# rahul-rwat/ESMStereo

Measured on AMD Instinct MI355X. Metric: stereo pairs/sec at 384×1248 maxdisp=192; EPE vs reference, higher is better.
Workload: dtype f32; 1 GPU; hot path: cost volume -> 3D stems -> 3D hourglass -> regression -> ESM upsampler (models/ESMStereo.py:700-745), ESMStereo-S gwc 384x1248 md192 B1; variant=S, cv=gwc, global_batch=1, height=384, width=1248, maxdisp=192, parallelism=dp1, graph=True

## Files before the change

### esmstereo_amd/blocks.py

```python
from __future__ import annotations

from typing import List, Optional, Sequence, Tuple

import torch
import torch.nn as nn
import torch.nn.functional as F

from .engine import (ACT_GELU, ACT_NONE, CONVT1X1_PAIRED, FORK_ENABLED, SC11_ENABLED, Ctx, PackedConv,
                     convt_1x1_supported, eager_emit, forked_packs, pack_conv, pack_shuffle_tail, pair2_auto,
                     param_token, run_conv, run_conv_forked, run_convt_1x1, run_pair2, run_shuffle_conv,
                     run_shuffle_tail, run_side_partial, shuffle_conv_pre_supported, shuffle_conv_supported)
from .mixer import FMBlock

__all__ = ["BasicConv", "Conv2x", "aggregation", "up_refinement", "upsample4", "upsample8", "upsample16"]


class BasicConv(nn.Module):

    def __init__(self, in_channels: int, out_channels: int, deconv: bool = False, is_3d: bool = False,
                 bn: bool = True, gelu: bool = True, **kwargs) -> None:
        super().__init__()
        self.gelu = gelu
        self.use_bn = bn
        kinds = {(False, False): nn.Conv2d, (False, True): nn.ConvTranspose2d,
                 (True, False): nn.Conv3d, (True, True): nn.ConvTranspose3d}
        self.conv = kinds[(bool(is_3d), bool(deconv))](in_channels, out_channels, bias=False, **kwargs)
        self.bn = (nn.BatchNorm3d if is_3d else nn.BatchNorm2d)(out_channels)
        self._esm = None

    def packed(self) -> PackedConv:
        tok = param_token(self.conv, self.bn) + (self.use_bn, self.gelu)
        if self._esm is None or self._esm[0] != tok:
            self._esm = (tok, pack_conv(self.conv, self.bn if self.use_bn else None,
                                        ACT_GELU if self.gelu else ACT_NONE))
        return self._esm[1]

    def emit(self, ctx: Ctx, srcs: Sequence[torch.Tensor], **epi) -> torch.Tensor:
        return run_conv(ctx, self.packed(), srcs, tag=getattr(self, "_esm_name", "BasicConv"), **epi)

    def forward(self, x: torch.Tensor) -> torch.Tensor:
        return self.emit(Ctx(x.device), [x])


class Conv2x(nn.Module):

    def __init__(self, in_channels: int, out_channels: int, deconv: bool = False, is_3d: bool = False,
                 concat: bool = True, keep_concat: bool = True, bn: bool = True, gelu: bool = True,
                 keep_dispc: bool = False) -> None:
        super().__init__()
        self.concat = concat
        self.is_3d = is_3d
        if deconv and is_3d and keep_dispc:
            self.conv1 = BasicConv(in_channels, out_channels, deconv, is_3d, bn=True, gelu=True,
                                   kernel_size=(1, 4, 4), stride=(1, 2, 2), padding=(0, 1, 1))
        else:
            k = (4 if not is_3d else (4, 4, 4)) if deconv else 3
            self.conv1 = BasicConv(in_channels, out_channels, deconv, is_3d, bn=True, gelu=True, kernel_size=k,
                                   stride=2, padding=1)
        mul = (2 if keep_concat else 1) if concat else 1
        cin2 = out_channels * 2 if concat else out_channels
        self.conv2 = BasicConv(cin2, out_channels * mul, False, is_3d, bn, gelu, kernel_size=3, stride=1, padding=1)

    def forward(self, x: torch.Tensor, rem: torch.Tensor) -> torch.Tensor:
        x = self.conv1(x)
        if x.shape != rem.shape:
            x = F.interpolate(x, size=(rem.shape[-2], rem.shape[-1]), mode="nearest")
        if self.concat:
            return self.conv2.emit(Ctx(x.device), [x, rem]) if x.shape[1] % 4 == 0 and rem.shape[1] % 4 == 0 \
                else self.conv2(torch.cat((x, rem), 1))
        return self.conv2(x + rem)


def _bc(cin: int, cout: int, is_3d: bool, k: int = 3, s: int = 1, p: int = 1, **kw) -> BasicConv:
    return BasicConv(cin, cout, is_3d=is_3d, kernel_size=k, stride=s, padding=p, **kw)


def _up(cin: int, cout: int, is_3d: bool, last: bool = False) -> BasicConv:
    return BasicConv(cin, cout, deconv=True, is_3d=is_3d, bn=not last, gelu=not last, kernel_size=4, padding=1,
                     stride=2)


def _pair(ctx: Ctx, first: BasicConv, srcs: Sequence[torch.Tensor], second, second_packed: Optional[PackedConv] = None,
          regress: Optional[torch.Tensor] = None, **kw) -> torch.Tensor:
    n0 = getattr(first, "_esm_name", "BasicConv")
    n1 = getattr(second, "_esm_name", "conv") if second is not None else "conv"
    pb = second_packed if second_packed is not None else second.packed()
    if not kw:
        return run_pair2(ctx, first.packed(), srcs, pb, tags=(n0, n1), regress=regress)
    if regress is not None:
        raise ValueError("_pair: regress with an epilogue")
    mid = run_conv(ctx, first.packed(), srcs, tag=n0)
    return run_conv(ctx, pb, [mid], tag=n1, **kw)


def _crop_like(t: torch.Tensor, ref: torch.Tensor) -> torch.Tensor:
    idx = (slice(None), slice(None)) + tuple(slice(0, n) for n in ref.shape[2:])
    return t[idx]


class _Hourglass(nn.Module):

    is_3d = False

    def _build(self, c_in: int, c1: int, c2: int, c3: int, cat0: int, cat1: int) -> None:
        d3 = self.is_3d
        self.conv1 = nn.Sequential(_bc(c_in, c1, d3, s=2), _bc(c1, c1, d3))
        self.conv2 = nn.Sequential(_bc(c1, c2, d3, s=2), _bc(c2, c2, d3))
        self.conv3 = nn.Sequential(_bc(c2, c3, d3, s=2), _bc(c3, c3, d3))
        self.conv3_up = _up(c3, c2, d3)
        self.conv2_up = _up(c2, c1, d3)
        self.conv1_up = _up(c1, 1, d3, last=True)
        self.agg_0 = nn.Sequential(_bc(cat0, c2, d3, k=1, p=0), _bc(c2, c2, d3))
        self.agg_1 = nn.Sequential(_bc(cat1, c1, d3, k=1, p=0), _bc(c1, c1, d3))

    def _emit(self, ctx: Ctx, x: Optional[torch.Tensor], extra0: Sequence[torch.Tensor] = (),
              extra1: Sequence[torch.Tensor] = (), crop1: bool = True, c10: Optional[torch.Tensor] = None,
              c11: Optional[torch.Tensor] = None, **last) -> torch.Tensor:
        if c11 is not None:
            c1 = c11
        elif c10 is not None:
            c1 = self.conv1[1].emit(ctx, [c10])
        else:
            c1 = _pair(ctx, self.conv1[0], [x], self.conv1[1])
        c2 = _pair(ctx, self.conv2[0], [c1], self.conv2[1])
        c3 = _pair(ctx, self.conv3[0], [c2], self.conv3[1])
        a0 = self._up_agg(ctx, self.conv3_up, c3, self.agg_0, [c2, *extra0], True)
        a1 = self._up_agg(ctx, self.conv2_up, a0, self.agg_1, [c1, *extra1], crop1)
        return self.conv1_up.emit(ctx, [a1], **last)

    def _up_agg(self, ctx: Ctx, up: BasicConv, x: torch.Tensor, agg: nn.Sequential, skip: Sequence[torch.Tensor],
                crop: bool) -> torch.Tensor:
        ref = skip[0]
        if not crop and tuple(2 * v for v in x.shape[2:]) != tuple(ref.shape[2:]):
            raise RuntimeError(f"Sizes of tensors must match except in dimension 1. Expected size "
                               f"{2 * x.shape[2]} but got size {ref.shape[2]} for tensor number 1 in the list.")
        pa, pb = up.packed(), agg[0].packed()
        u_shape = tuple(2 * v for v in x.shape[2:])
        n0 = getattr(up, "_esm_name", "convT")
        n1 = getattr(agg[0], "_esm_name", "agg.0")
        paired = pair2_auto(pb, agg[1].packed(), [ref]) if not self.is_3d else False
        fork = FORK_ENABLED and not self.is_3d and len(skip) == 2 and agg[0].use_bn and int(skip[0].shape[1]) % 4 == 0
        if fork:
            cm = pa.cout + int(skip[0].shape[1])
            p_side, p_main = forked_packs(agg[0], agg[0].conv, agg[0].bn, ACT_GELU if agg[0].gelu else ACT_NONE, cm,
                                          int(skip[1].shape[1]))
            if convt_1x1_supported(pa, p_main, skip[:1]) and all(u >= r for u, r in zip(u_shape, ref.shape[2:])):
                part = run_side_partial(ctx, p_side, skip[1], n1, cm)
                h = run_convt_1x1(ctx, pa, [x], p_main, skip[:1], tags=(n0, n1), pre=part)
                ctx.meta[-1]["split"] = (0, cm)
                return agg[1].emit(ctx, [h])
            u = _crop_like(up.emit(ctx, [x]), ref)
            part = run_side_partial(ctx, p_side, skip[1], n1, cm)
            h = run_conv(ctx, p_main, [u, skip[0]], pre=part, tag=n1)
            ctx.meta[-1].update(layer=n1, split=(0, cm))
            return agg[1].emit(ctx, [h])
        if convt_1x1_supported(pa, pb, skip) and all(u >= r for u, r in zip(u_shape, ref.shape[2:])) and \
                (CONVT1X1_PAIRED or not paired):
            h = run_convt_1x1(ctx, pa, [x], pb, skip, tags=(n0, n1))
            return agg[1].emit(ctx, [h])
        u = _crop_like(up.emit(ctx, [x]), ref)
        return _pair(ctx, agg[0], [u, *skip], agg[1])


class aggregation(_Hourglass):

    is_3d = True

    def __init__(self, in_channels: int, add_channel: int) -> None:
        super().__init__()
        c0, a = in_channels, add_channel
        self._build(c0, c0 + a, c0 + 2 * a, c0 + 4 * a, 2 * (c0 + 2 * a), 2 * (c0 + a))

    def emit(self, ctx: Ctx, x: torch.Tensor, **last) -> torch.Tensor:
        return self._emit(ctx, x, crop1=True, **last)

    def forward(self, x: torch.Tensor) -> torch.Tensor:
        return eager_emit(x.device, self.emit, x)


class up_refinement(_Hourglass):

    is_3d = False

    def __init__(self, C: int, cf1: int, cf2: int) -> None:
        super().__init__()
        self._build(1, C, C, C, 2 * C + cf1, 2 * C + cf2)

    def emit(self, ctx: Ctx, disp: Optional[torch.Tensor], left_f1x: torch.Tensor, left_f2x: torch.Tensor,
             c10: Optional[torch.Tensor] = None, c11: Optional[torch.Tensor] = None, **last) -> torch.Tensor:
        return self._emit(ctx, disp, extra0=[left_f1x], extra1=[left_f2x], crop1=False, c10=c10, c11=c11, **last)

    def forward(self, disp: torch.Tensor, left_f1x: torch.Tensor, left_f2x: torch.Tensor) -> torch.Tensor:
        return eager_emit(disp.device, self.emit, disp, left_f1x, left_f2x)




def _dm(c: int) -> nn.Sequential:
    return nn.Sequential(_bc(1, c, False, k=5), _bc(c, c, False), _bc(c, c, False), _bc(c, c, False, k=1, p=1))


def _spx(cin: int, c: int, cout: int) -> nn.Sequential:
    return nn.Sequential(_bc(cin, c, False), nn.Conv2d(c, cout, 3, 1, 1, bias=False), nn.BatchNorm2d(cout), nn.GELU())


def _shuffle_up(nf: int, r: int) -> nn.Sequential:
    return nn.Sequential(nn.Conv2d(nf, nf * r * r, 1, 1, 0), nn.PixelShuffle(r), nn.SiLU(inplace=True))


class _ESMUpsampler(nn.Module):

    STAGES: Tuple = ()
    N_FEATS = 8

    def __init__(self) -> None:
        super().__init__()
        nf = self.N_FEATS
        for i, (tag, C, catc, spx_out, r, cf1, cf2, *_src) in enumerate(self.STAGES):
            setattr(self, f"dm{tag}", _dm(C))
            setattr(self, f"spx_{tag}", _spx(C + catc, C, spx_out))
            if i == 0:
                self.to_feat = nn.Conv2d(C, nf, 3, 1, 1, bias=False)
                self.blocks = nn.Sequential(*[FMBlock(nf, 7, 2) for _ in range(2)])
            setattr(self, f"upsampling{tag[:-1]}", _shuffle_up(nf, r))
            setattr(self, f"tail{tag}", nn.Conv2d(nf, 1, 3, 1, 1))
            setattr(self, f"ref{tag}", up_refinement(C, cf1, cf2))
        self._esm = None

    def _packed(self):
        tok = param_token(*self.modules())
        if self._esm is None or self._esm[0] != tok:
            p = {"to_feat": pack_conv(self.to_feat)}
            for (tag, _C, _cat, _spx, r, *_r) in self.STAGES:
                spx = getattr(self, f"spx_{tag}")
                p[f"spx1_{tag}"] = pack_conv(spx[1], spx[2], ACT_GELU)
                p[f"up_{tag}"] = pack_shuffle_tail(getattr(self, f"upsampling{tag[:-1]}")[0], getattr(self, f"tail{tag}"),
                                                   r)
            self._esm = (tok, p)
        return self._esm[1]

    def emit(self, ctx: Ctx, feats: Sequence[torch.Tensor], init_disp: torch.Tensor, final_scale: float = 1.0,
             scaled_copies: Optional[float] = None, init_cost: Optional[torch.Tensor] = None) -> List[torch.Tensor]:
        p = self._packed()
        me = getattr(self, "_esm_name", "upsample")
# ... 88 lines not shown
```

### esmstereo_amd/csrc/conv_pair2.hip

```cpp
#include "conv_direct.h"

namespace esm {
namespace conv {
namespace {

constexpr int kP2Threads = 256;
constexpr int kHintPairReg = 1 << 29;

__device__ __forceinline__ float regress_px(const float* __restrict__ cp, int D, int sc) {
#pragma clang fp contract(off)
    float acc = 0.f;
    for (int d0 = 0; d0 < D; d0 += 16) {
        float v[16];
#pragma unroll
        for (int k = 0; k < 16; ++k) v[k] = d0 + k < D ? cp[(d0 + k) * sc] : 0.f;
#pragma unroll
        for (int k = 0; k < 16; ++k)
            if (d0 + k < D) acc = acc + v[k] * static_cast<float>(d0 + k);
    }
    return acc;
}

template <int KA, int SA, int KB, int TH>
struct P2Geo {
// ... 185 lines not shown
        const bool ok = yb < bd.Ho && xb < bd.Wo && n < VB;
        const __amdgpu_buffer_rsrc_t ro = __builtin_amdgcn_make_buffer_rsrc(
            bd.out + b * bd.ob, static_cast<short>(0),
            4 * ((bd.Cout - 1) * static_cast<int>(bd.oc) + (bd.Ho - 1) * static_cast<int>(bd.oh) + bd.Wo), 0x00020000);
#pragma unroll
        for (int j = 0; j < 4; ++j) {
            const int co = 4 * kq + j;
            const float v = act_t<ESM_ACT_GELU>((acc[0][j] + acc[1][j]) * ep[32 + co] + ep[48 + co], 0);
            const unsigned o = (ok && co < bd.Cout) ? 4u * (co * static_cast<int>(bd.oc) + yb * static_cast<int>(bd.oh) + xb)
                                                    : kOOB;
            store_b32(__float_as_uint(v), ro, static_cast<int>(o), 0);
        }
    }
}

template <int KA, int SA, int KB, int TH, int CINMAX, bool REG = false>
int launch_p2(const esm_conv_desc& a, const esm_conv_desc& b, hipStream_t s) {
    using G = P2Geo<KA, SA, KB, TH>;
    const size_t lds = sizeof(float) * (static_cast<size_t>(CINMAX) * G::ICS + KA * KA * CINMAX * 16 + KB * KB * 256 +
                                        16 * G::ACS + 64);
    constexpr int VB = 16 - KB + 1;
    const dim3 grid(ceil_div(b.Wo, VB), ceil_div(b.Ho, TH), a.B);
    if (grid.y > 65535u || grid.z > 65535u) return arg_error("conv pair: grid too large");
    if constexpr (REG) {
        const int pr = b.ph + a.ph, pc = b.pw + a.pw;
        if (pr < 0 || pc < 0 || TH > G::IR - pr || VB > G::IC - pc ||
            (static_cast<int>(grid.y) - 1) * TH - pr + G::IR < a.Hi || (static_cast<int>(grid.x) - 1) * VB - pc + G::IC < a.Wi)
            return arg_error("conv pair: regressed map not covered by the tiles");
    }
    hipLaunchKernelGGL((pair2_kernel<KA, SA, KB, TH, CINMAX, REG>), grid, dim3(kP2Threads), lds, s, a, b);
    return check_launch("conv pair");
}

template <int KA, int SA, int KB>
int launch_p2_k(const esm_conv_desc& a, const esm_conv_desc& b, hipStream_t s) {
    const long long tiles4 = static_cast<long long>(ceil_div(b.Wo, 16 - KB + 1)) * ceil_div(b.Ho, 4) * a.B;
    const int thsel = (b.hint >> 26) & 3;
    const bool small = thsel ? thsel == 1 : tiles4 < 256;
    const bool tall = thsel == 3 && a.Cin <= 16;
    if constexpr (KA == 5 && KB == 3) {
        if (a.hint & kHintPairReg) {
            if (tall) return launch_p2<KA, SA, KB, 8, 4, true>(a, b, s);
            return small ? launch_p2<KA, SA, KB, 2, 4, true>(a, b, s) : launch_p2<KA, SA, KB, 4, 4, true>(a, b, s);
        }
    }
    if (tall) return a.Cin <= 4 ? launch_p2<KA, SA, KB, 8, 4>(a, b, s) : launch_p2<KA, SA, KB, 8, 16>(a, b, s);
    if (a.Cin <= 4) return small ? launch_p2<KA, SA, KB, 2, 4>(a, b, s) : launch_p2<KA, SA, KB, 4, 4>(a, b, s);
    if (a.Cin <= 16) return small ? launch_p2<KA, SA, KB, 2, 16>(a, b, s) : launch_p2<KA, SA, KB, 4, 16>(a, b, s);
    if (a.Cin <= 32) return small ? launch_p2<KA, SA, KB, 2, 32>(a, b, s) : launch_p2<KA, SA, KB, 4, 32>(a, b, s);
    if constexpr (KA == 1) {
        if (a.Cin > 48) return small ? launch_p2<KA, SA, KB, 2, 64>(a, b, s) : launch_p2<KA, SA, KB, 4, 64>(a, b, s);
    }
    return small ? launch_p2<KA, SA, KB, 2, 48>(a, b, s) : launch_p2<KA, SA, KB, 4, 48>(a, b, s);
}

}

bool pair2_lds_ok(const esm_conv_desc& a, const esm_conv_desc& b) {
    const bool a3 = a.kd > 1 || a.Di > 1 || a.Do > 1, b3 = b.kd > 1 || b.Di > 1 || b.Do > 1;
    if (a3 || b3 || a.transposed || b.transposed || a.shuffle > 1 || b.shuffle > 1) return false;
    if (a.Cout != 16 || a.Cin < 1 || a.Cin > (a.kh == 1 ? 64 : 48) || b.Cin != 16 || b.Cout < 1 || b.Cout > 16)
        return false;
    if (!((a.kh == 3 && (a.stride == 1 || a.stride == 2)) || ((a.kh == 1 || a.kh == 5) && a.stride == 1))) return false;
    if (a.ph != a.pw || b.ph != b.pw || b.stride != 1 || (b.kh != 1 && b.kh != 3)) return false;
    if (a.act != ESM_ACT_GELU || b.act != ESM_ACT_GELU) return false;
    if (a.mul || a.res || a.up || a.out2 || a.post_scale != 1.f) return false;
    if (b.mul || b.res || b.up || b.out2 || b.post_scale != 1.f || !b.out) return false;
    if (b.Hi != a.Ho || b.Wi != a.Wo || b.B != a.B) return false;
    if (b.Ho != b.Hi + 2 * b.ph - b.kh + 1 || b.Wo != b.Wi + 2 * b.pw - b.kw + 1) return false;
    if (a.nsrc > 1)
        for (int i = 0; i < a.nsrc; ++i)
            if (a.src[i].C % 4) return false;
    if (a.hint & kHintPairReg) {
        if (a.kh != 5 || b.kh != 3 || a.Cin != 1 || a.nsrc != 1 || a.src[0].C < 1 || !a.out || a.out == b.out)
            return false;
        if (static_cast<long long>(a.src[0].C) * a.src[0].sc >= (1LL << 31) || a.src[0].sh >= (1 << 28)) return false;
    }
    const long long last = (b.Cout - 1) * b.oc + (b.Ho - 1) * b.oh + b.Wo;
    return 4 * last < static_cast<long long>(kOOB) && b.oc < (1 << 28) && b.oh < (1 << 28);
}

bool pairk_ok(const esm_conv_desc& a, const esm_conv_desc& b);
int launch_pairk(const esm_conv_desc& a, const esm_conv_desc& b, hipStream_t s);

constexpr int kHintPairK = 1 << 28;

bool pair2_ok(const esm_conv_desc& a, const esm_conv_desc& b) {
    if (a.pre || b.pre) return false;
    return pair2_lds_ok(a, b) || pairk_ok(a, b);
}

int launch_pair2(const esm_conv_desc& a, const esm_conv_desc& b, hipStream_t s) {
    if (a.pre || b.pre) return arg_error("conv pair: a partial sum (pre) is not supported on either conv");
    const bool lds = pair2_lds_ok(a, b);
    if (((b.hint & kHintPairK) || !lds) && !(a.hint & kHintPairReg) && pairk_ok(a, b)) return launch_pairk(a, b, s);
    if (!lds) return arg_error("conv pair: unsupported pair");
    if (a.kh == 5) return b.kh == 3 ? launch_p2_k<5, 1, 3>(a, b, s) : launch_p2_k<5, 1, 1>(a, b, s);
    if (a.kh == 1) return b.kh == 3 ? launch_p2_k<1, 1, 3>(a, b, s) : launch_p2_k<1, 1, 1>(a, b, s);
    if (a.stride == 2) return b.kh == 3 ? launch_p2_k<3, 2, 3>(a, b, s) : launch_p2_k<3, 2, 1>(a, b, s);
    return b.kh == 3 ? launch_p2_k<3, 1, 3>(a, b, s) : launch_p2_k<3, 1, 1>(a, b, s);
}

}
}

extern "C" int esm_conv_pair2_f32(const esm_conv_desc* a, const esm_conv_desc* b, void* stream) {
    if (!a || !b) return esm::arg_error("conv pair: null descriptor");
    return esm::conv::launch_pair2(*a, *b, esm::as_stream(stream));
}
```

### esmstereo_amd/engine.py

```python
from __future__ import annotations

import contextlib
import ctypes
import json
import math
import os
import threading
from dataclasses import dataclass
from typing import Dict, List, Optional, Sequence, Tuple

import torch

from . import _lib
from ._lib import (ACT_GELU, ACT_NONE, ACT_RELU, ACT_RELU6, ACT_SIGMOID, ACT_SILU, EsmConfDesc, EsmConvDesc, EsmShuffleConvDesc,
                   EsmShuffleTailDesc, EsmSmixDesc, check, lib)

__all__ = ["Ctx", "PackedConv", "pack_conv", "run_conv", "run_smix", "run_fmnet", "run_shuffle_tail", "pack_shuffle_tail",
           "ACT_NONE", "ACT_GELU", "ACT_SILU", "ACT_RELU", "ACT_SIGMOID", "ACT_RELU6", "run_dwconv", "cached_pack", "run_convt_1x1",
           "convt_1x1_supported", "pack_conv_split", "run_conv_forked",
           "forked_packs", "run_side_partial"]


def _rup(x: int, m: int) -> int:
    return (x + m - 1) // m * m
# ... 747 lines not shown


def forked_packs(owner: torch.nn.Module, conv: torch.nn.Module, bn: Optional[torch.nn.Module], act: int, cm: int,
                 cs: int) -> Tuple[PackedConv, PackedConv]:
    def build():
        return (pack_conv_split(conv, None, act, cm, cm + cs), pack_conv_split(conv, bn, act, 0, cm))
    return cached_pack(owner, f"fork{cm}", [conv, bn], build)


def run_side_partial(ctx: Ctx, p_side: PackedConv, side: torch.Tensor, tag: str, cm: int) -> torch.Tensor:
    with ctx.side():
        part = run_conv(ctx, p_side, [side], tag=tag + "[side]")
    ctx.meta[-1].update(layer=tag, split=(cm, cm + p_side.cin))
    ctx.join_next()
    return part


def run_conv_forked(ctx: Ctx, owner: torch.nn.Module, conv: torch.nn.Module, bn: Optional[torch.nn.Module], act: int,
                    main: Sequence[torch.Tensor], side: torch.Tensor, tag: str = "conv") -> torch.Tensor:
    cm = sum(int(t.shape[1]) for t in main)
    p_side, p_main = forked_packs(owner, conv, bn, act, cm, int(side.shape[1]))
    part = run_side_partial(ctx, p_side, side, tag, cm)
    out = run_conv(ctx, p_main, list(main), pre=part, tag=tag)
    ctx.meta[-1].update(layer=tag, split=(0, cm))
    return out


PAIR_REGRESS_ENABLED = _ab("ESM_PAIR_REGRESS", "1") != "0"
PAIR2_TH = {sel: tuple(x for x in _ab(f"ESM_PAIR2_TH{n}", "").split(",") if x)
            for sel, n in ((1, 2), (2, 4), (3, 8))}
HINT_PAIR_REGRESS = 1 << 29


def run_pair2(ctx: Ctx, pa: PackedConv, srcs: Sequence[torch.Tensor], pb: PackedConv,
              tags: Tuple[str, str] = ("convA", "convB"), force: bool = False,
              regress: Optional[torch.Tensor] = None, ksplit: Optional[bool] = None,
              out: Optional[torch.Tensor] = None) -> torch.Tensor:
    take = pair2_supported(pa, pb, srcs) if force else pair2_auto(pa, pb, srcs)
    if ksplit is None:
        ksplit = take and regress is None and ((not force and pairk_auto(pa, pb, srcs)) or
                                               not _pair2_lds_supported(pa, pb, srcs))
    elif take and not (pairk_supported if ksplit else _pair2_lds_supported)(pa, pb, srcs):
        raise ValueError("conv pair: the requested form does not run this pair")
    if regress is not None:
        B_, D_, H_, W_ = (int(v) for v in regress.shape)
        init = srcs[0]
        fuse = (take and PAIR_REGRESS_ENABLED and len(srcs) == 1 and pa.k == 5 and pb.k == 3 and pa.cin == 1
                and regress.stride(3) == 1 and tuple(init.shape) == (B_, 1, H_, W_) and init.stride(3) == 1)
        if not fuse:
            ctx.regression(0, regress, init, B_, D_, H_, W_)
            regress = None
    if not take:
        return run_conv(ctx, pb, [run_conv(ctx, pa, srcs, tag=tags[0])], out, tag=tags[1])
    da, _, ma = _conv_desc(ctx, pa, srcs, tag=tags[0], alloc_out=False)
    da.hint &= ~HINT_PAIR_REGRESS
    B = int(srcs[0].shape[0])
    geo = (B, pa.cout) + ((int(da.Do),) if pa.nd == 3 else ()) + (int(da.Ho), int(da.Wo))
    virt = srcs[0].as_strided(geo, (0,) * (len(geo) - 1) + (1,))
    db, out, mb = _conv_desc(ctx, pb, [virt], out, tag=tags[1])
    db.hint &= ~((3 << 26) | HINT_PAIRK)
    if ksplit:
        db.hint |= HINT_PAIRK
    for sel, subs in PAIR2_TH.items():
        if any(x in tags[0] for x in subs):
            db.hint |= sel << 26
    mid = 4 * B * pa.cout * int(da.Ho) * int(da.Wo) * (int(da.Do) if pa.nd == 3 else 1)
    name = f"{tags[0]}+{tags[1].rsplit('.', 1)[-1]}"
    flops, byts, reads, writes = ma["flops"] + mb["flops"], ma["bytes"] - mid + mb["bytes"] - mid, ma["reads"], mb["writes"]
    if regress is not None:
        require_on(init.device, "pair regression", regress)
        st = regress.stride()
        da.src[0].ptr, da.src[0].C = regress.data_ptr(), D_
        da.src[0].sb, da.src[0].sc, da.src[0].sh = st[0], st[1], st[2]
        da.out = init.data_ptr()
        da.ob, da.oc, da.oh = init.stride(0), init.stride(1), init.stride(2)
        da.hint |= HINT_PAIR_REGRESS
        ctx.hold(regress, init)
        name = "disparity_regression+" + name
        flops += 2 * B_ * D_ * H_ * W_
        byts += 4 * B_ * D_ * H_ * W_
        reads, writes = _spans(regress), writes + _spans(init)
    ctx.meta.append(dict(name=name, kind="conv_pair", flops=flops, bytes=byts, shape=f"pair {ma['shape']} + {mb['shape']}",
                         reads=reads, writes=writes, key=ma["key"] + " | " + mb["key"], hint=0))
    ctx.pair2(da, db)
    return out


def run_dwconv(ctx: Ctx, x: torch.Tensor, w: torch.Tensor, scale: Optional[torch.Tensor], shift: Optional[torch.Tensor],
               k: int, stride: int, pad: int, act: int, tag: str = "dwconv",
               out: Optional[torch.Tensor] = None) -> torch.Tensor:
    if stride <= 0 or k <= 0 or not 0 <= pad < k:
        raise ValueError("dwconv: stride and K must be positive, 0 <= pad < K")
    if x.dim() != 4 or x.stride(3) != 1:
        raise ValueError("dwconv: a [B, C, H, W] input with unit W stride")
    require_device(x, "dwconv input")
    B, C, H, W = (int(v) for v in x.shape)
    Ho, Wo = (H + 2 * pad - k) // stride + 1, (W + 2 * pad - k) // stride + 1
    if out is None:
        out = ctx.empty(B, C, Ho, Wo)
    elif tuple(out.shape) != (B, C, Ho, Wo) or out.stride(3) != 1:
        raise ValueError("dwconv: output must be [B, C, Ho, Wo] with unit W stride")
    require_on(x.device, "dwconv", x, w, scale, shift, out)
    d = _lib.EsmDwconvDesc()
    d.x, d.xb, d.xc, d.xh = x.data_ptr(), x.stride(0), x.stride(1), x.stride(2)
    d.w = w.data_ptr()
    d.scale = scale.data_ptr() if scale is not None else None
    d.shift = shift.data_ptr() if shift is not None else None
    d.out, d.ob, d.oc, d.oh = out.data_ptr(), out.stride(0), out.stride(1), out.stride(2)
    d.B, d.C, d.H, d.W, d.K, d.stride, d.pad, d.act, d.Ho, d.Wo = B, C, H, W, k, stride, pad, act, Ho, Wo
    ctx.meta.append(dict(name=tag, kind="dwconv", flops=2 * B * C * Ho * Wo * k * k,
                         bytes=4 * (x.numel() + out.numel() + C * k * k), reads=_spans(x), writes=_spans(out)))
    ctx.dwconv(d)
    return out


@dataclass
class SmixStage:
    ln_w: torch.Tensor
    fc0_w: torch.Tensor
    fc0_b: torch.Tensor
    fc2_w: torch.Tensor
    fc2_b: torch.Tensor


def run_smix(ctx: Ctx, x: torch.Tensor, stages: Sequence[SmixStage], *, dw: Optional[Tuple[torch.Tensor, torch.Tensor]] = None,
             res: Optional[torch.Tensor] = None, out: Optional[torch.Tensor] = None, tag: str = "smix") -> torch.Tensor:
    require_device(x, "smix input")
    if not x.is_contiguous():
        raise ValueError("smix: input must be contiguous")
    B, C, H, W = (int(v) for v in x.shape)
    if out is None:
        out = ctx.empty(B, C, H, W)
    d = EsmSmixDesc()
    d.x, d.out = x.data_ptr(), out.data_ptr()
    if res is not None:
        require_device(res, "smix residual")
        if not res.is_contiguous() or res.shape != x.shape:
            raise ValueError("smix: residual must be contiguous and shaped like the input")
        d.res = res.data_ptr()
    if dw is not None:
        d.dw_w, d.dw_b = dw[0].data_ptr(), dw[1].data_ptr()
        d.dw_k = int(dw[0].shape[-1])
    if len(stages) > _lib.SMIX_MAX_STAGES:
        raise ValueError("smix: at most 2 stages per launch")
    require_on(x.device, "smix", x, out, res, *(dw or ()),
               *[t for st in stages for t in (st.ln_w, st.fc0_w, st.fc0_b, st.fc2_w, st.fc2_b)])
    d.nstages = len(stages)
    for i, st in enumerate(stages):
        d.stage[i].ln_w = st.ln_w.data_ptr()
        d.stage[i].fc0_w, d.stage[i].fc0_b = st.fc0_w.data_ptr(), st.fc0_b.data_ptr()
        d.stage[i].fc2_w, d.stage[i].fc2_b = st.fc2_w.data_ptr(), st.fc2_b.data_ptr()
        ctx.hold(st.ln_w, st.fc0_w, st.fc0_b, st.fc2_w, st.fc2_b)
    d.B, d.C, d.H, d.W = B, C, H, W
    ctx.hold(x, out, res, *(dw or ()))
    npix = B * H * W
    ctx.meta.append(dict(name=tag, kind="smix", flops=npix * (2 * C * C * len(stages) + (2 * C * d.dw_k ** 2 if dw else 0)),
                         bytes=4 * npix * C * (3 if res is not None else 2), shape=f"C{C} {H}x{W} dw{d.dw_k}",
                         reads=_spans(x, res), writes=_spans(out)))
    ctx.smix(d)
    return out


FM2_MIN_PIX = int(_ab("ESM_FM2_MIN_PIX", "16384"))


def run_fmnet(ctx: Ctx, x: torch.Tensor, stages: Sequence[SmixStage], dw0: Tuple[torch.Tensor, torch.Tensor],
# ... 227 lines not shown
```

Before: 3296 pairs/s.

## Fuse last 2-D hourglass 3x3 conv with transposed-conv k4s2 head in one kernel

Adds a fused HIP kernel that runs the final 3x3 BN+GELU conv (≤16→16 channels) with MFMA, keeps its 16-channel output tile in shared memory, and immediately applies the 16→1 transposed conv k4 s2 head with its bilinear-add and scaled-copy epilogue. The 2-D hourglass now defers the agg_1[1] conv and dispatches this pair when shapes and pixel count allow. This removes the write and re-read of the intermediate 16-channel feature map and one kernel launch. In exchange it adds halo recomputation at tile borders, a large shared-memory tile and more code paths.

```diff
diff --git a/esmstereo_amd/blocks.py b/esmstereo_amd/blocks.py
--- a/esmstereo_amd/blocks.py
+++ b/esmstereo_amd/blocks.py
@@ -8,7 +8,8 @@
 
 from .engine import (ACT_GELU, ACT_NONE, CONVT1X1_PAIRED, FORK_ENABLED, SC11_ENABLED, Ctx, PackedConv,
                      convt_1x1_supported, eager_emit, forked_packs, pack_conv, pack_shuffle_tail, pair2_auto,
-                     param_token, run_conv, run_conv_forked, run_convt_1x1, run_pair2, run_shuffle_conv,
+                     pair_head_auto, param_token, run_conv, run_conv_forked, run_convt_1x1, run_pair2, run_pair_head,
+                     run_shuffle_conv,
                      run_shuffle_tail, run_side_partial, shuffle_conv_pre_supported, shuffle_conv_supported)
 from .mixer import FMBlock
 
@@ -112,6 +113,7 @@
         self.conv1_up = _up(c1, 1, d3, last=True)
         self.agg_0 = nn.Sequential(_bc(cat0, c2, d3, k=1, p=0), _bc(c2, c2, d3))
         self.agg_1 = nn.Sequential(_bc(cat1, c1, d3, k=1, p=0), _bc(c1, c1, d3))
+        object.__setattr__(self.agg_1, "conv1_up", self.conv1_up)
 
     def _emit(self, ctx: Ctx, x: Optional[torch.Tensor], extra0: Sequence[torch.Tensor] = (),
               extra1: Sequence[torch.Tensor] = (), crop1: bool = True, c10: Optional[torch.Tensor] = None,
@@ -124,12 +126,21 @@
             c1 = _pair(ctx, self.conv1[0], [x], self.conv1[1])
         c2 = _pair(ctx, self.conv2[0], [c1], self.conv2[1])
         c3 = _pair(ctx, self.conv3[0], [c2], self.conv3[1])
-        a0 = self._up_agg(ctx, self.conv3_up, c3, self.agg_0, [c2, *extra0], True)
-        a1 = self._up_agg(ctx, self.conv2_up, a0, self.agg_1, [c1, *extra1], crop1)
+        a0, _ = self._up_agg(ctx, self.conv3_up, c3, self.agg_0, [c2, *extra0], True)
+        head = not self.is_3d and set(last) <= {"up", "up_f", "post_scale", "out2", "post_scale2"} and \
+            pair_head_auto(self.agg_1[1].packed(), self.conv1_up.packed(), [c1])
+        a1, open_ = self._up_agg(ctx, self.conv2_up, a0, self.agg_1, [c1, *extra1], crop1, defer=head)
+        if open_:
+            return run_pair_head(ctx, self.agg_1[1].packed(), [a1], self.conv1_up.packed(),
+                                 tags=(getattr(self.agg_1[1], "_esm_name", "agg_1.1"),
+                                       getattr(self.conv1_up, "_esm_name", "conv1_up")), **last)
         return self.conv1_up.emit(ctx, [a1], **last)
 
     def _up_agg(self, ctx: Ctx, up: BasicConv, x: torch.Tensor, agg: nn.Sequential, skip: Sequence[torch.Tensor],
-                crop: bool) -> torch.Tensor:
+                crop: bool, defer: bool = False):
+        def tail(h):
+            return (h, True) if defer else (agg[1].emit(ctx, [h]), False)
+
         ref = skip[0]
         if not crop and tuple(2 * v for v in x.shape[2:]) != tuple(ref.shape[2:]):
             raise RuntimeError(f"Sizes of tensors must match except in dimension 1. Expected size "
@@ -148,18 +159,20 @@
                 part = run_side_partial(ctx, p_side, skip[1], n1, cm)
                 h = run_convt_1x1(ctx, pa, [x], p_main, skip[:1], tags=(n0, n1), pre=part)
                 ctx.meta[-1]["split"] = (0, cm)
-                return agg[1].emit(ctx, [h])
+                return tail(h)
             u = _crop_like(up.emit(ctx, [x]), ref)
             part = run_side_partial(ctx, p_side, skip[1], n1, cm)
             h = run_conv(ctx, p_main, [u, skip[0]], pre=part, tag=n1)
             ctx.meta[-1].update(layer=n1, split=(0, cm))
-            return agg[1].emit(ctx, [h])
+            return tail(h)
         if convt_1x1_supported(pa, pb, skip) and all(u >= r for u, r in zip(u_shape, ref.shape[2:])) and \
                 (CONVT1X1_PAIRED or not paired):
             h = run_convt_1x1(ctx, pa, [x], pb, skip, tags=(n0, n1))
-            return agg[1].emit(ctx, [h])
+            return tail(h)
         u = _crop_like(up.emit(ctx, [x]), ref)
-        return _pair(ctx, agg[0], [u, *skip], agg[1])
+        if defer and not paired:
+            return agg[0].emit(ctx, [u, *skip]), True
+        return _pair(ctx, agg[0], [u, *skip], agg[1]), False
 
 
 class aggregation(_Hourglass):
diff --git a/esmstereo_amd/csrc/conv_headt.hip b/esmstereo_amd/csrc/conv_headt.hip
--- /dev/null
+++ b/esmstereo_amd/csrc/conv_headt.hip
@@ -0,0 +1,203 @@
+#include "conv_wide_rows.h"
+
+namespace esm {
+
+int conv_check(const esm_conv_desc& a);
+
+namespace conv {
+namespace {
+
+constexpr int kHtThreads = 256;
+
+template <int R, int S>
+struct HtGeo {
+    static constexpr int NL = 16 * S;
+    static constexpr int P = NL + 2;
+    static constexpr int CS0 = (R + 2) * P;
+    static constexpr int CS = CS0 + ((16 - CS0 % 64) + 64) % 64;
+};
+
+template <int NG, int R, int S, bool WIN>
+__global__ void __launch_bounds__(kHtThreads) headt_kernel(const esm_conv_desc a, const esm_conv_desc bd, const float* wbase,
+                                                           int wspan, int d0) {
+    using G = HtGeo<R, S>;
+    constexpr int KS = 4 / S, NL = G::NL, P = G::P, CS = G::CS;
+    __shared__ float tile[16 * CS];
+    __shared__ __attribute__((aligned(16))) float wb[16 * 16];
+    const int tid = static_cast<int>(threadIdx.x);
+    const int lane = tid & 63;
+    const int wave = __builtin_amdgcn_readfirstlane(tid >> 6);
+    const int n16 = lane & 15, kq = lane >> 4;
+    const Blk3 bk_ = xcd_block((bd.hint & kHintXcd) != 0);
+    const int a0 = bk_.y * R;
+    const int c0 = bk_.x * (NL - 1);
+    const int b = bk_.z;
+
+    {
+        const int c = tid >> 4, k = tid & 15;
+        wb[tid] = bd.w[(static_cast<long long>(k) * bd.cin_pad + c) * bd.cout_pad];
+        constexpr int NBR = P + 2 * (R + 1);
+        for (int e = tid; e < 16 * NBR; e += kHtThreads) {
+            const int ch = e / NBR, q = e - ch * NBR;
+            const int cell = q < P ? q : (1 + (q - P) / 2) * P + (((q - P) & 1) ? P - 1 : 0);
+            tile[ch * CS + cell] = 0.f;
+        }
+    }
+
+    float scl[4], shf[4];
+    const int strip = wave / KS;
+    const int xa = c0 + strip * 16 + n16;
+    float* trow = tile + (4 * kq) * CS + P + 1 + strip * 16 + n16;
+    wide_rows<3, NG, 1, R + 1, KS, WIN>(
+        a, wbase, wspan, d0, 0, 0, lane, wave, c0 + strip * 16, a0, b,
+        [&]() {
+#pragma unroll
+            for (int j = 0; j < 4; ++j) {
+                scl[j] = a.scale[4 * kq + j];
+                shf[j] = a.shift[4 * kq + j];
+            }
+        },
+        [](int, int) { return floatx4{0.f, 0.f, 0.f, 0.f}; },
+        [&](int r, const floatx4(&acc)[1]) {
+            const bool inside = a0 + r < a.Ho && xa < a.Wo;
+#pragma unroll
+            for (int j = 0; j < 4; ++j) {
+                const float v = act_t<ESM_ACT_GELU>(acc[0][j] * scl[j] + shf[j], 0);
+                trow[j * CS + r * P] = inside ? v : 0.f;
+            }
+        });
+    __syncthreads();
+
+    const int l = lane & (NL - 1);
+    const int x = c0 + l;
+    const bool vx0 = x < a.Wo && (l > 0 || bk_.x == 0);
+    const bool vx1 = x < a.Wo && l < NL - 1;
+    const __amdgpu_buffer_rsrc_t ro = __builtin_amdgcn_make_buffer_rsrc(
+        bd.out + b * bd.ob, static_cast<short>(0), 4 * ((bd.Ho - 1) * static_cast<int>(bd.oh) + bd.Wo), 0x00020000);
+    const __amdgpu_buffer_rsrc_t ro2 = __builtin_amdgcn_make_buffer_rsrc(
+        (bd.out2 ? bd.out2 : bd.out) + b * bd.ob, static_cast<short>(0), 4 * ((bd.Ho - 1) * static_cast<int>(bd.oh) + bd.Wo),
+        0x00020000);
+    const bool vec = ((bd.ob | bd.oh) & 1) == 0 && (reinterpret_cast<uintptr_t>(bd.out) & 7) == 0 &&
+                     (reinterpret_cast<uintptr_t>(bd.out2) & 7) == 0;
+    constexpr int UPW = 64 / NL;
+#pragma unroll 1
+    for (int u0 = wave * UPW; u0 <= R; u0 += 4 * UPW) {
+        const int u = u0 + (UPW > 1 ? lane / NL : 0);
+        const int p = u < R ? u : -1;
+        const int oy1 = 2 * (a0 + p) + 1;
+        const bool vy[2] = {p >= 0 && oy1 < bd.Ho, oy1 + 1 < bd.Ho};
+        if (u > R || (p < 0 && bk_.y != 0) || !(vx0 || vx1) || !(vy[0] || vy[1])) continue;
+        float o[2][2] = {{0.f, 0.f}, {0.f, 0.f}};
+        const float* tp = tile + (p + 1) * P + l;
+#pragma unroll 2
+        for (int c = 0; c < 16; ++c) {
+            float t[2][3];
+#pragma unroll
+            for (int i = 0; i < 2; ++i)
+#pragma unroll
+                for (int j = 0; j < 3; ++j) t[i][j] = tp[c * CS + i * P + j];
+            const floatx4* wc = reinterpret_cast<const floatx4*>(wb + 16 * c);
+#pragma unroll
+            for (int dy = 0; dy < 2; ++dy)
+#pragma unroll
+                for (int qw = 0; qw < 2; ++qw) {
+                    const floatx4 w4 = wc[(1 - dy) * 2 + qw];
+#pragma unroll
+                    for (int th = 0; th < 2; ++th)
+#pragma unroll
+                        for (int tw = 0; tw < 2; ++tw) o[dy][qw] = fmaf(w4[th * 2 + tw], t[1 - th][1 + qw - tw], o[dy][qw]);
+                }
+        }
+#pragma unroll
+        for (int dy = 0; dy < 2; ++dy) {
+            if (!vy[dy]) continue;
+            const int oy = oy1 + dy;
+            const float v0 = vx0 ? conv_finish(bd, o[dy][0], b, 0, 0, oy, 2 * x) : 0.f;
+            const float v1 = vx1 ? conv_finish(bd, o[dy][1], b, 0, 0, oy, 2 * x + 1) : 0.f;
+            const int off = 4 * (oy * static_cast<int>(bd.oh) + 2 * x);
+            if (vec && vx0 && vx1) {
+                typedef unsigned int u32x2 __attribute__((ext_vector_type(2)));
+                const u32x2 s1 = {__float_as_uint(v0 * bd.post_scale), __float_as_uint(v1 * bd.post_scale)};
+                __builtin_amdgcn_raw_buffer_store_b64(s1, ro, off, 0, kStoreAux);
+                if (bd.out2) {
+                    const u32x2 s2 = {__float_as_uint(v0 * bd.post_scale2), __float_as_uint(v1 * bd.post_scale2)};
+                    __builtin_amdgcn_raw_buffer_store_b64(s2, ro2, off, 0, kStoreAux);
+                }
+            } else {
+                if (vx0) {
+                    store_b32(__float_as_uint(v0 * bd.post_scale), ro, off, 0);
+                    if (bd.out2) store_b32(__float_as_uint(v0 * bd.post_scale2), ro2, off, 0);
+                }
+                if (vx1) {
+                    store_b32(__float_as_uint(v1 * bd.post_scale), ro, off + 4, 0);
+                    if (bd.out2) store_b32(__float_as_uint(v1 * bd.post_scale2), ro2, off + 4, 0);
+                }
+            }
+        }
+    }
+}
+
+template <int NG, int R, int S>
+int launch_ht(const esm_conv_desc& a, const esm_conv_desc& b, hipStream_t s) {
+    constexpr int NL = 16 * S;
+    const dim3 grid(ceil_div(a.Wo, NL - 1), ceil_div(a.Ho, R), static_cast<unsigned>(a.B));
+    if (grid.y > 65535u || grid.z > 65535u) return arg_error("conv pair (head): grid too large");
+    const float* base = nullptr;
+    int span = 0, dl[ESM_MAX_SRC] = {0, 0, 0};
+    if (source_window(a, &base, &span, dl))
+        hipLaunchKernelGGL((headt_kernel<NG, R, S, true>), grid, dim3(kHtThreads), 0, s, a, b, base, span, dl[0]);
+    else
+        hipLaunchKernelGGL((headt_kernel<NG, R, S, false>), grid, dim3(kHtThreads), 0, s, a, b, base, span, 0);
+    return check_launch("conv pair (head)");
+}
+
+template <int NG>
+int launch_ht_g(const esm_conv_desc& a, const esm_conv_desc& b, hipStream_t s) {
+    if ((b.hint >> 26) & 3) return arg_error("conv pair (head): unknown block selector (hint bits 26-27)");
+    return launch_ht<NG, 8, 2>(a, b, s);
+}
+
+const char* headt_why(const esm_conv_desc& a, const esm_conv_desc& b) {
+    const bool a3 = a.kd > 1 || a.Di > 1 || a.Do > 1, b3 = b.kd > 1 || b.Di > 1 || b.Do > 1;
+    if (a3 || b3) return "2-D layers only";
+    if (a.pre || b.pre) return "a partial sum (pre) is not supported on either conv";
+    if (a.transposed || a.kh != 3 || a.kw != 3 || a.stride != 1 || a.ph != 1 || a.pw != 1)
+        return "the first conv must be 3x3, stride 1, padding 1";
+    if (a.nsrc != 1 || !a.src[0].ptr) return "the first conv takes one source";
+    if (a.Cin < 1 || a.Cin > 16 || a.Cout != 16) return "the first conv must have <= 16 inputs and 16 outputs";
+    if (a.act != ESM_ACT_GELU || !a.scale || !a.shift || a.mul || a.res || a.up || a.out2 || a.shuffle > 1 ||
+        a.post_scale != 1.f)
+        return "the first conv's epilogue must be plain BN + GELU";
+    if (!b.transposed || b.kh != 4 || b.kw != 4 || b.stride != 2 || b.ph != 1 || b.pw != 1)
+        return "the head must be a transposed conv k4 s2 p1";
+    if (b.Cin != 16 || b.Cout != 1 || b.cin_pad < 16) return "the head must be 16 -> 1";
+    if (b.scale || b.act != ESM_ACT_NONE || b.mul || b.res || b.shuffle > 1)
+        return "the head takes a bias, the bilinear add and the scaled copies only (no BN, activation, mul, res)";
+    if (b.B != a.B || b.Hi != a.Ho || b.Wi != a.Wo || b.Ho != 2 * b.Hi || b.Wo != 2 * b.Wi)
+        return "the head's input extent must be the first conv's output extent";
+    if (b.up && (b.up_f <= 0 || b.up_h * b.up_f != b.Ho || b.up_w * b.up_f != b.Wo))
+        return "bilinear source extent x factor must equal the output extent";
+    if (!b.out || b.ob < 0 || b.oh < b.Wo) return "bad output strides";
+    const long long last = static_cast<long long>(b.Ho - 1) * b.oh + b.Wo;
+    if (4 * last >= static_cast<long long>(kOOB) || b.oh >= (1 << 28)) return "output span too large";
+    if (!direct_ok(a)) return "source span too large";
+    return "";
+}
+
+}
+
+bool headt_ok(const esm_conv_desc& a, const esm_conv_desc& b) { return headt_why(a, b)[0] == 0; }
+
+int launch_headt(const esm_conv_desc& a, const esm_conv_desc& b, hipStream_t s) {
+    esm_conv_desc ac = a;
+    if (!ac.out) ac.out = b.out;
+    int rc = conv_check(ac);
+    if (rc == ESM_OK) rc = conv_check(b);
+    if (rc != ESM_OK) return rc;
+    const char* why = headt_why(a, b);
+    if (why[0]) return arg_error(std::string("conv pair (head): ") + why);
+    return a.Cin <= 8 ? launch_ht_g<2>(a, b, s) : launch_ht_g<4>(a, b, s);
+}
+
+}
+}
diff --git a/esmstereo_amd/csrc/conv_pair2.hip b/esmstereo_amd/csrc/conv_pair2.hip
--- a/esmstereo_amd/csrc/conv_pair2.hip
+++ b/esmstereo_amd/csrc/conv_pair2.hip
@@ -291,16 +291,20 @@
 
 bool pairk_ok(const esm_conv_desc& a, const esm_conv_desc& b);
 int launch_pairk(const esm_conv_desc& a, const esm_conv_desc& b, hipStream_t s);
+bool headt_ok(const esm_conv_desc& a, const esm_conv_desc& b);
+int launch_headt(const esm_conv_desc& a, const esm_conv_desc& b, hipStream_t s);
 
 constexpr int kHintPairK = 1 << 28;
 
 bool pair2_ok(const esm_conv_desc& a, const esm_conv_desc& b) {
     if (a.pre || b.pre) return false;
+    if (b.transposed) return headt_ok(a, b);
     return pair2_lds_ok(a, b) || pairk_ok(a, b);
 }
 
 int launch_pair2(const esm_conv_desc& a, const esm_conv_desc& b, hipStream_t s) {
     if (a.pre || b.pre) return arg_error("conv pair: a partial sum (pre) is not supported on either conv");
+    if (b.transposed) return launch_headt(a, b, s);
     const bool lds = pair2_lds_ok(a, b);
     if (((b.hint & kHintPairK) || !lds) && !(a.hint & kHintPairReg) && pairk_ok(a, b)) return launch_pairk(a, b, s);
     if (!lds) return arg_error("conv pair: unsupported pair");
diff --git a/esmstereo_amd/csrc/conv_wide_rows.h b/esmstereo_amd/csrc/conv_wide_rows.h
--- /dev/null
+++ b/esmstereo_amd/csrc/conv_wide_rows.h
@@ -0,0 +1,143 @@
+#pragma once
+
+#include "conv_direct.h"
+
+namespace esm {
+namespace conv {
+
+template <int K, int NG, int MT, int R, int KS, bool WIN, class AW, class Init, class Fin>
+__device__ __forceinline__ void wide_rows(const esm_conv_desc& a, const float* wbase, int wspan, int d0, int d1, int d2,
+                                          int lane, int wave, int x0, int y0, int b, AW&& after_weights, Init&& init,
+                                          Fin&& finish) {
+    constexpr int NR = R + K - 1;
+    constexpr int NGW = (NG + KS - 1) / KS;
+    static_assert(KS == 1 || KS == 2, "K split: two waves");
+    const int n16 = lane & 15, kq = lane >> 4;
+    const int kh = KS == 2 ? (wave & 1) : 0;
+    const int gb = kh * NGW;
+    const int cob = 0;
+
+    float wv[K * K][NGW][MT];
+    {
+        const __amdgpu_buffer_rsrc_t wrs = __builtin_amdgcn_make_buffer_rsrc(
+            const_cast<float*>(a.w), static_cast<short>(0), 4 * K * K * a.cin_pad * a.cout_pad, 0x00020000);
+        const unsigned wl = 4u * (kq * a.cout_pad + cob + n16);
+#pragma unroll
+        for (int t = 0; t < K * K; ++t)
+#pragma unroll
+            for (int g = 0; g < NGW; ++g)
+#pragma unroll
+                for (int mt = 0; mt < MT; ++mt)
+                    wv[t][g][mt] = buf_load_s(wrs, wl, 4 * ((t * a.cin_pad + 4 * (gb + g)) * a.cout_pad + 16 * mt));
+    }
+    after_weights();
+
+    const int sh = static_cast<int>(a.src[0].sh);
+    const int ns = a.nsrc;
+    const int lo1 = a.src[0].C, lo2 = a.src[0].C + (ns > 1 ? a.src[1].C : 0);
+    auto src_rsrc = [&](const esm_src& q) __attribute__((always_inline)) {
+        return __builtin_amdgcn_make_buffer_rsrc(const_cast<float*>(q.ptr + b * q.sb), static_cast<short>(0),
+                                                 4 * ((q.C - 1) * static_cast<int>(q.sc) + (a.Hi - 1) * sh + a.Wi),
+                                                 0x00020000);
+    };
+    const __amdgpu_buffer_rsrc_t rs0 = WIN ? __builtin_amdgcn_make_buffer_rsrc(const_cast<float*>(wbase), static_cast<short>(0),
+                                                                               wspan, 0x00020000)
+                                           : src_rsrc(a.src[0]);
+    const __amdgpu_buffer_rsrc_t rs1 = !WIN && ns > 1 ? src_rsrc(a.src[1]) : rs0;
+    const __amdgpu_buffer_rsrc_t rs2 = !WIN && ns > 2 ? src_rsrc(a.src[2]) : rs0;
+    const int xo = x0 + n16;
+    int gs[NGW];
+    unsigned vo[NGW][K];
+#pragma unroll
+    for (int g = 0; g < NGW; ++g) {
+        const int cg = 4 * (gb + g);
+        gs[g] = cg < lo1 ? 0 : (cg < lo2 ? 1 : 2);
+        const int c = cg + kq;
+        const int s = gs[g];
+        const int cl = c - (s == 0 ? 0 : (s == 1 ? lo1 : lo2));
+        const long long sb = s == 0 ? a.src[0].sb : (s == 1 ? a.src[1].sb : a.src[2].sb);
+        const long long sc = s == 0 ? a.src[0].sc : (s == 1 ? a.src[1].sc : a.src[2].sc);
+        const int dl = s == 0 ? d0 : (s == 1 ? d1 : d2);
+#pragma unroll
+        for (int dx = 0; dx < K; ++dx) {
+            const int xi = xo - a.pw + dx;
+            const bool ok = c < a.Cin && xo < a.Wo && xi >= 0 && xi < a.Wi;
+            if constexpr (WIN)
+                vo[g][dx] = ok ? static_cast<unsigned>(dl + 4 * (b * sb + cl * sc + xi)) : kOOB;
+            else
+                vo[g][dx] = ok ? 4u * static_cast<unsigned>(cl * static_cast<int>(sc) + xi) : kOOB;
+        }
+    }
+    auto load_row = [&](float (&dst)[NGW][K], int r) {
+        const int yi = y0 - a.ph + r;
+        const int roff = (yi >= 0 && yi < a.Hi) ? 4 * yi * sh : static_cast<int>(kOOB);
+#pragma unroll
+        for (int g = 0; g < NGW; ++g)
+#pragma unroll
+            for (int dx = 0; dx < K; ++dx)
+                dst[g][dx] = buf_load_s(WIN ? rs0 : (gs[g] == 0 ? rs0 : (gs[g] == 1 ? rs1 : rs2)), vo[g][dx], roff);
+    };
+
+    floatx4 acc[R][MT];
+#pragma unroll
+    for (int r = 0; r < R; ++r)
+#pragma unroll
+        for (int mt = 0; mt < MT; ++mt)
+            acc[r][mt] = kh == 0 ? init(r, mt) : floatx4{0.f, 0.f, 0.f, 0.f};
+
+    constexpr int PF = R >= 4 ? 2 : 1;
+    constexpr int NB = PF + 1;
+    float bin[NB][NGW][K];
+#pragma unroll
+    for (int r = 0; r < PF; ++r) load_row(bin[r], r);
+#pragma unroll
+    for (int r = 0; r < NR; ++r) {
+        if (r + PF < NR) load_row(bin[(r + PF) % NB], r + PF);
+        __builtin_amdgcn_sched_barrier(0);
+#pragma unroll
+        for (int g = 0; g < NGW; ++g)
+#pragma unroll
+            for (int dx = 0; dx < K; ++dx)
+#pragma unroll
+                for (int dy = 0; dy < K; ++dy) {
+                    const int ro = r - dy;
+                    if (ro < 0 || ro >= R) continue;
+#pragma unroll
+                    for (int mt = 0; mt < MT; ++mt)
+                        acc[ro][mt] = __builtin_amdgcn_mfma_f32_16x16x4f32(wv[dy * K + dx][g][mt], bin[r % NB][g][dx],
+                                                                           acc[ro][mt], 0, 0, 0);
+                }
+        if (KS == 1 && r - (K - 1) >= 0) finish(r - (K - 1), acc[r - (K - 1)]);
+    }
+    if constexpr (KS == 2) {
+        constexpr int RH = (R + 1) / 2;
+        __shared__ float xch[4][RH * MT * 4][64];
+#pragma unroll
+        for (int r = 0; r < R; ++r) {
+            if ((r < RH) != (kh == 0)) {
+#pragma unroll
+                for (int mt = 0; mt < MT; ++mt)
+#pragma unroll
+                    for (int j = 0; j < 4; ++j) xch[wave][((r % RH) * MT + mt) * 4 + j][lane] = acc[r][mt][j];
+            }
+        }
+        __syncthreads();
+        const int partner = wave ^ 1;
+#pragma unroll
+        for (int r = 0; r < R; ++r) {
+            if ((r < RH) == (kh == 0)) {
+#pragma unroll
+                for (int mt = 0; mt < MT; ++mt)
+#pragma unroll
+                    for (int j = 0; j < 4; ++j) {
+                        const float p = xch[partner][((r % RH) * MT + mt) * 4 + j][lane];
+                        acc[r][mt][j] = kh == 0 ? acc[r][mt][j] + p : p + acc[r][mt][j];
+                    }
+                finish(r, acc[r]);
+            }
+        }
+    }
+}
+
+}
+}
diff --git a/esmstereo_amd/engine.py b/esmstereo_amd/engine.py
--- a/esmstereo_amd/engine.py
+++ b/esmstereo_amd/engine.py
@@ -853,6 +853,53 @@
         reads, writes = _spans(regress), writes + _spans(init)
     ctx.meta.append(dict(name=name, kind="conv_pair", flops=flops, bytes=byts, shape=f"pair {ma['shape']} + {mb['shape']}",
                          reads=reads, writes=writes, key=ma["key"] + " | " + mb["key"], hint=0))
+    ctx.pair2(da, db)
+    return out
+
+
+PAIR_HEAD_ENABLED = _ab("ESM_PAIR_HEAD", "1") != "0"
+PAIR_HEAD_MIN_PIX = int(_ab("ESM_PAIR_HEAD_MIN_PIX", "65536"))
+PAIR_HEAD_TILES = {0: (8, 2)}
+
+
+def pair_head_supported(pa: PackedConv, pb: PackedConv, srcs: Sequence[torch.Tensor]) -> bool:
+    if pa.nd != 2 or pb.nd != 2 or pa.transposed or not pb.transposed or len(srcs) != 1:
+        return False
+    if (pa.k, pa.stride, pa.pad) != (3, 1, 1) or (pb.k, pb.stride, pb.pad) != (4, 2, 1):
+        return False
+    if not 1 <= pa.cin <= 16 or pa.cout != 16 or pa.act != ACT_GELU or pa.scale is None or pa.shift is None:
+        return False
+    return pb.cin == 16 and pb.cout == 1 and pb.scale is None and pb.act == ACT_NONE
+
+
+def pair_head_auto(pa: PackedConv, pb: PackedConv, srcs: Sequence[torch.Tensor]) -> bool:
+    if not PAIR_HEAD_ENABLED or not pair_head_supported(pa, pb, srcs):
+        return False
+    return int(srcs[0].shape[0]) * math.prod(_pair_out(pa, srcs)) >= PAIR_HEAD_MIN_PIX
+
+
+def run_pair_head(ctx: Ctx, pa: PackedConv, srcs: Sequence[torch.Tensor], pb: PackedConv,
+                  tags: Tuple[str, str] = ("convA", "head"), tile: Optional[int] = None,
+                  out: Optional[torch.Tensor] = None, **epi) -> torch.Tensor:
+    if not pair_head_supported(pa, pb, srcs) or set(epi) - {"up", "up_f", "post_scale", "out2", "post_scale2"}:
+        raise ValueError("conv pair (head): unsupported layers or epilogue")
+    sel = 0 if tile is None else int(tile)
+    if sel not in PAIR_HEAD_TILES:
+        raise ValueError("conv pair (head): unknown tile selector")
+    da, _, ma = _conv_desc(ctx, pa, srcs, tag=tags[0], alloc_out=False)
+    da.hint &= ~HINT_PAIR_REGRESS
+    B = int(srcs[0].shape[0])
+    geo = (B, pa.cout, int(da.Ho), int(da.Wo))
+    virt = srcs[0].as_strided(geo, (0, 0, 0, 1))
+    db, out, mb = _conv_desc(ctx, pb, [virt], out, tag=tags[1], **epi)
+    db.hint = (db.hint & ~((3 << 26) | HINT_PAIRK)) | (sel << 26)
+    mid = 4 * B * pa.cout * int(da.Ho) * int(da.Wo)
+    up = epi.get("up")
+    extra = 4 * up.numel() if up is not None else 0
+    name = f"{tags[0]}+{tags[1].rsplit('.', 1)[-1]}"
+    ctx.meta.append(dict(name=name, kind="conv_pair", flops=ma["flops"] + mb["flops"],
+                         bytes=ma["bytes"] - mid + mb["bytes"] - extra - mid, shape=f"pair {ma['shape']} + {mb['shape']}",
+                         reads=ma["reads"] + _spans(up), writes=mb["writes"], key=ma["key"] + " | " + mb["key"], hint=0))
     ctx.pair2(da, db)
     return out
 
```

Measured after the change: 3321 pairs/s (median of 6 runs). Within noise of the previous version (+0.8%).
